# tlroy/thermalporous

Hardware: AMD Instinct MI355X
Metric: Newton steps/s, SPE10 60x220x85 two-phase (FGMRES its/s in config) (higher is better)
Workload: dtype f64; 1 GPU; BASELINE config 4: two-phase 3D SPE10-like 60x220x85, wells+heaters, pc_cptr, maxdt 0.1 day; grid 60x220x85 (synthetic default_rng(10) field); FGMRES rtol 1e-08; timed at dt = maxdt after an untimed spin-up along the reference's dt ramp; newton_its=84, fgmres_its=2689, failed_solves=0, slabs=none

## Files before the change

include/thermalporous_hip.h:

```cpp
#ifndef THERMALPOROUS_HIP_H
#define THERMALPOROUS_HIP_H

#include <stdint.h>

#ifdef __cplusplus
extern "C" {
#endif

typedef struct tp_ctx tp_ctx;

typedef struct tp_grid {
    int32_t n0, n1, n2;
    int32_t gn2, off2;
    double  h[3];
    int32_t gaxis;
    int32_t nphase;
    int32_t rank, nranks;
} tp_grid;

typedef struct tp_params {
    double ko, kw, kr, c_v_w, c_v_o, c_r, rho_r, p_inj, p_prod, T_inj, T_prod, API, p_ref, g,
           S_o, U, rate;
} tp_params;

// ... 54 lines not shown
int tp_set_field(tp_ctx *ctx, const char *name, const double *host, int64_t n);
int tp_finalize_fields(tp_ctx *ctx);
int tp_set_sources(tp_ctx *ctx, int32_t n, const tp_source *entries);

int tp_set_state(tp_ctx *ctx, const double *u_host);
int tp_get_state(tp_ctx *ctx, double *u_host);
int tp_set_old_state(tp_ctx *ctx, const double *u_host);
int tp_set_dt(tp_ctx *ctx, double dt);
int tp_get_old_state(tp_ctx *ctx, double *u_host);
int tp_restore_state(tp_ctx *ctx);
int tp_saturation_range(tp_ctx *ctx, double *smin, double *smax);
int tp_clamp_saturation(tp_ctx *ctx);

int tp_residual(tp_ctx *ctx, double *norm2);
int tp_jacobian(tp_ctx *ctx);
int tp_get_residual(tp_ctx *ctx, double *host);
int tp_export_jacobian(tp_ctx *ctx, double *host);
int tp_export_schur(tp_ctx *ctx, double *host);
int tp_well_rates(tp_ctx *ctx, double *rate, double *water_rate, double *oil_rate);

int tp_vec_create(tp_ctx *ctx, int32_t *id);
int tp_vec_set(tp_ctx *ctx, int32_t id, const double *host);
int tp_vec_get(tp_ctx *ctx, int32_t id, double *host);
int tp_vec_copy_residual(tp_ctx *ctx, int32_t id);

typedef void (*tp_ksp_monitor_fn)(int32_t its, double rnorm, const double *field_norms, int32_t nfields, void *user);
int tp_set_ksp_monitor(tp_ctx *ctx, tp_ksp_monitor_fn cb, void *user);

int tp_vec_create_batch(tp_ctx *ctx, int32_t n, int32_t *first_id);
int tp_vec_dot_batch(tp_ctx *ctx, int32_t first, int32_t n, int32_t w, double *out);
int tp_vec_axpy_batch(tp_ctx *ctx, int32_t first, int32_t n, const double *coef, int32_t w);
int tp_vec_norm2(tp_ctx *ctx, int32_t x, double *out);
int tp_spmv(tp_ctx *ctx, int32_t x, int32_t y);
int tp_pc_setup(tp_ctx *ctx);
int tp_pc_apply(tp_ctx *ctx, int32_t x, int32_t y);
int tp_stage1_update(tp_ctx *ctx);
int tp_stage1_apply(tp_ctx *ctx, int32_t x, int32_t y);
int tp_ilu0_factor(tp_ctx *ctx);
int tp_ilu0_solve(tp_ctx *ctx, int32_t x, int32_t y);
int tp_ilu_layout(tp_ctx *ctx, int32_t out[8]);
int tp_amg_setup(tp_ctx *ctx, int32_t which);
int tp_amg_vcycle(tp_ctx *ctx, int32_t which, int32_t field_b, int32_t b, int32_t field_x, int32_t x);
int tp_schur_apply(tp_ctx *ctx, int32_t x, int32_t y);

int tp_inner_stats(tp_ctx *ctx, int64_t *applies, int64_t *its, int64_t *unconverged);

int tp_fgmres(tp_ctx *ctx, int32_t b, int32_t x, int32_t *its, int32_t *reason, double *rnorm);
int tp_newton_solve(tp_ctx *ctx, tp_solve_info *info);

int tp_time_kernel(tp_ctx *ctx, int32_t which, int32_t reps, double *ms_avg);
int tp_amg_info(tp_ctx *ctx, int32_t which, int32_t *nlevels, double *op_complexity);
int tp_amg_trunc(tp_ctx *ctx, int32_t which, int32_t *level, double *ratio0);
int tp_amg_layout(tp_ctx *ctx, int32_t which, int32_t *dist_levels, int32_t *axes, int32_t cap, int32_t *naxes);

#ifdef __cplusplus
}
#endif
#endif
```

thermalporous_amd/csrc/tp_amg.hip:

```cpp
#include "tp_common.hpp"
#include <algorithm>
#include <cstdlib>

namespace tp {

template <class R>
struct StencilT {
    R *base;
    long slot_stride;
    __host__ __device__ const R *slot(int s) const { return base + (long)s * slot_stride; }
};

__device__ __forceinline__ void cell_ijk(const GridDev &g, long tid, int &i0, int &i1, int &i2) {
    const unsigned t = (unsigned)tid, np = (unsigned)g.np, n0 = (unsigned)g.n0;
    const unsigned q2 = t / np, rem = t - q2 * np, q1 = rem / n0;
    i2 = (int)q2;
    i1 = (int)q1;
    i0 = (int)(rem - q1 * n0);
}

template <class R>
__global__ void k_amg_weights(GridDev g, StencilT<R> A, int axis, double omega, R *wm, R *wp, R *invd,
                              unsigned long long *ratio_slots) {
    const long tid = (long)blockIdx.x * blockDim.x + threadIdx.x;
// ... 469 lines not shown
    if (tid >= Lf.g.nown) return;
    out[Lf.g.np + tid] = prolong_jacobi_cell(Lf, gc, b, x, ec, tid);
}

template <class R>
__global__ __launch_bounds__(256) void k_amg_restrict2(LevelDevT<R> L0, LevelDevT<R> L1, GridDev g2, const double *r,
                                                       double *rc) {
    const long tid = xcd_tid();
    if (tid >= g2.nown) return;
    rc[g2.np + tid] = restrict2_cell(L0, L1, g2, r, tid);
}
template <class R>
__global__ __launch_bounds__(256) void k_amg_prolong2_jacobi(LevelDevT<R> L0, LevelDevT<R> L1, GridDev g2, const double *b,
                                                             const double *e2, double *out) {
    const long tid = xcd_tid();
    if (tid >= L0.g.nown) return;
    out[L0.g.np + tid] = prolong2_jacobi_cell(L0, L1, g2, b, e2, tid);
}

template <class R>
__global__ __launch_bounds__(256) void k_amg_resid(LevelDevT<R> L, const double *__restrict__ b,
                                                   const double *__restrict__ x, double *__restrict__ r) {
    const long tid = xcd_tid();
    if (tid >= L.g.nown) return;
    r[L.g.np + tid] = resid_at(L, b, x, L.g.np + tid);
}
template <class R>
__global__ __launch_bounds__(256) void k_amg_restrict(LevelDevT<R> Lf, GridDev gc, const double *__restrict__ r,
                                                      double *__restrict__ rc) {
    const long tid = xcd_tid();
    if (tid >= gc.nown) return;
    rc[gc.np + tid] = restrict_cell(Lf, gc, r, tid);
}
template <class R>
__global__ __launch_bounds__(256) void k_amg_prolong_set(LevelDevT<R> Lf, GridDev gc, const double *__restrict__ ec,
                                                         double *__restrict__ out) {
    const long tid = xcd_tid();
    if (tid >= Lf.g.nown) return;
    int i0, i1, i2;
    cell_ijk(Lf.g, tid, i0, i1, i2);
    out[Lf.g.np + tid] = prolong_val<R, false>(Lf, gc, ec, i0, i1, i2);
}
template <class R>
__global__ __launch_bounds__(256) void k_amg_prolong_add(LevelDevT<R> Lf, GridDev gc, const double *__restrict__ ec,
                                                         double *x) {
    const long tid = xcd_tid();
    if (tid >= Lf.g.nown) return;
    int i0, i1, i2;
    cell_ijk(Lf.g, tid, i0, i1, i2);
    x[Lf.g.np + tid] += prolong_val<R, false>(Lf, gc, ec, i0, i1, i2);
}

template <class R>
__global__ __launch_bounds__(1024) void k_amg_tail(const LevelDevT<R> *lv, int l0, int nlev_all, int trunc, int ncoarse,
                                                   const double *Minv, const double *b_top, double *e_top,
                                                   int lds_doubles) {
    const int nlev = trunc >= 0 ? trunc + 1 : nlev_all;
    extern __shared__ double dyn[];
    constexpr int T = 1024;
    const int t = threadIdx.x;
    static_assert(sizeof(LevelDevT<R>) % sizeof(long) == 0, "LevelDev must be a whole number of words");
    __shared__ long slv_raw[40 * sizeof(LevelDevT<R>) / sizeof(long)];
    {
        const int wpl = (int)(sizeof(LevelDevT<R>) / sizeof(long));
        const long *src = reinterpret_cast<const long *>(lv);
        for (int i = l0 * wpl + t; i < nlev * wpl; i += T) slv_raw[i] = src[i];
        if (lds_doubles > 0)
            for (int i = t; i < 4 * lds_doubles; i += T) dyn[i] = 0.0;
        __syncthreads();
    }
    if (lds_doubles > 0) {
        if (t == 0) {
            LevelDevT<R> *w = reinterpret_cast<LevelDevT<R> *>(slv_raw);
            long off = 0;
            for (int l = l0; l < nlev; ++l) {
                w[l].b = dyn + off;
                w[l].e = dyn + lds_doubles + off;
                w[l].x = dyn + 2 * lds_doubles + off;
                w[l].x2 = dyn + 3 * lds_doubles + off;
                off += w[l].g.ntot;
            }
        }
        __syncthreads();
    }
    lv = reinterpret_cast<const LevelDevT<R> *>(slv_raw);
    {
        double sink = 0.0;
        for (int l = l0; l < nlev; ++l) {
            const LevelDevT<R> &L = lv[l];
            for (long i = L.g.np + t; i < L.g.np + L.g.nown; i += T) {
#pragma unroll
                for (int k = 0; k < 7; ++k) sink += (double)L.op.slot(k)[i];
                sink += (double)L.invd[i];
                if (L.axis >= 0) sink += (double)L.wm[i] + (double)L.wp[i];
            }
        }
        if (trunc < 0)
            for (int i = t; i < ncoarse * ncoarse; i += T) sink += Minv[i];
        if (sink == 1.2345678e-300) e_top[0] = sink;
    }
    for (int l = l0; l < nlev - 1; ++l) {
        const LevelDevT<R> L = lv[l];
        const GridDev gc = lv[l + 1].g;
        const double *b = (l == l0) ? b_top : L.b;
        double *rc = lv[l + 1].b;
        if (L.pre == 0) {
            for (long i = t; i < gc.nown; i += T) rc[gc.np + i] = restrict_cell(L, gc, b, i);
            __syncthreads();
            continue;
        }
        double *cur = L.x, *oth = L.x2;
        for (long i = t; i < L.g.nown; i += T)
            cur[L.g.np + i] = L.pre >= 2 ? pre2_cell(L, b, i) : L.invd[L.g.np + i] * b[L.g.np + i];
        __syncthreads();
        for (int k = 2; k < L.pre; ++k) {
            for (long i = t; i < L.g.nown; i += T) oth[L.g.np + i] = jacobi_cell(L, b, cur, i);
            __syncthreads();
            double *tmp = cur; cur = oth; oth = tmp;
        }
        for (long i = t; i < gc.nown; i += T) rc[gc.np + i] = resid_restrict_cell(L, gc, b, cur, i);
        __syncthreads();
    }
    {
        const LevelDevT<R> Lc = lv[nlev - 1];
        const double *b = (nlev - 1 == l0) ? b_top : Lc.b;
        double *e = (nlev - 1 == l0) ? e_top : Lc.e;
        if (trunc >= 0) {
            for (long i = t; i < Lc.g.nown; i += T) e[Lc.g.np + i] = pre2_cell(Lc, b, i);
            __syncthreads();
        } else {
        const int grp = t >> 4, gl = t & 15;
        for (int r = grp; r < ncoarse; r += T >> 4) {
            double s = 0.0;
            for (int q = gl; q < ncoarse; q += 16) s += Minv[(long)r * ncoarse + q] * b[Lc.g.np + q];
            s += __shfl_xor(s, 8, 64);
            s += __shfl_xor(s, 4, 64);
            s += __shfl_xor(s, 2, 64);
            s += __shfl_xor(s, 1, 64);
            if (gl == 0) e[Lc.g.np + r] = s;
        }
        __syncthreads();
        }
    }
    for (int l = nlev - 2; l >= l0; --l) {
        const LevelDevT<R> L = lv[l];
        const GridDev gc = lv[l + 1].g;
        const double *b = (l == l0) ? b_top : L.b;
        double *out = (l == l0) ? e_top : L.e;
        const double *ec = lv[l + 1].e;
        const int extra = L.pre >= 2 ? L.pre - 2 : 0;
        const double *src = L.pre == 0 ? nullptr : ((extra % 2 == 0) ? L.x : L.x2);
        if (L.post == 0) {
            for (long i = t; i < L.g.nown; i += T) {
                int i0, i1, i2;
                cell_ijk(L.g, i, i0, i1, i2);
                out[L.g.np + i] = prolong_val(L, gc, ec, i0, i1, i2);
            }
            __syncthreads();
            continue;
        }
        double *dst = (L.post == 1) ? out : (src == L.x ? L.x2 : L.x);
        for (long i = t; i < L.g.nown; i += T) dst[L.g.np + i] = prolong_jacobi_cell(L, gc, b, src, ec, i);
        __syncthreads();
        for (int k = 1; k < L.post; ++k) {
            src = dst;
            dst = (k == L.post - 1) ? out : (src == L.x ? L.x2 : L.x);
            for (long i = t; i < L.g.nown; i += T) dst[L.g.np + i] = jacobi_cell(L, b, src, i);
            __syncthreads();
        }
    }
}

std::vector<std::pair<int, int>> rank_slabs(const tp_ctx *c) {
    std::vector<std::pair<int, int>> slabs(c->dist ? c->grid.nranks : 0);
    for (size_t r = 0; r < slabs.size(); ++r) slab_of(c, (int)r, slabs[r].first, slabs[r].second);
    return slabs;
}

AmgPlan amg_plan(const GridDev &g0, const double strength[3], const tp_options &o, int me,
                 const std::vector<std::pair<int, int>> &slabs, long gather_cells, long tail_cells) {
    AmgPlan P;
    int m[3] = {g0.n0, g0.n1, g0.n2};
    {
        int n[3] = {m[0], m[1], m[2]};
        double s[3];
        for (int a = 0; a < 3; ++a) s[a] = n[a] > 1 ? strength[a] : -1.0;
        while ((long)n[0] * n[1] * n[2] > std::max(1, o.amg_min_cells) && P.sched.size() < 40) {
            int best = -1;
            for (int a = 0; a < 3; ++a)
                if (n[a] > 1 && (best < 0 || s[a] > s[best])) best = a;
            if (best < 0) break;
            P.sched.push_back(best);
            n[best] = (n[best] + 1) / 2;
            for (int q = 0; q < 3; ++q) s[q] = (q == best) ? s[q] * 0.5 : s[q] * 2.0;
        }
    }
    std::vector<std::pair<int, int>> cur = slabs;
    if (cur.empty()) cur = {{0, m[2]}};
    bool still = !slabs.empty() && gather_cells >= 0;
    const int nu = std::max(1, o.amg_nu);
    for (size_t l = 0; l <= P.sched.size(); ++l) {
        AmgPlan::Level L;
        if (still) {
            int minp = 1 << 30;
            for (auto &q : cur) minp = std::min(minp, q.second - q.first);
            still = (long)m[0] * m[1] * m[2] > gather_cells && minp >= 2 && l < P.sched.size();
            if (still) P.dist_levels = (int)l + 1;
        }
        P.ranges.push_back(cur);
        L.g = still ? make_grid(m[0], m[1], cur[me].second - cur[me].first, m[2], cur[me].first)
                    : make_grid(m[0], m[1], m[2], m[2], 0);
        const bool full = (int)l < o.amg_full_levels;
        const bool small = L.g.np * (long)L.g.gn2 <= 1024;
        L.pre = full ? nu : std::max(0, o.amg_coarse_pre);
        L.post = full ? nu : std::max(1, small ? o.amg_tail_post : o.amg_coarse_post);
        if (o.amg_mid_skip && !full && !small && (((int)l - o.amg_full_levels) & 1)) { L.pre = 0; L.post = 0; }
        if (l < P.sched.size()) {
            L.axis = P.sched[l];
            m[L.axis] = (m[L.axis] + 1) / 2;
            if (L.axis == 2)
                for (auto &q : cur) q = {(q.first + 1) / 2, (q.second + 1) / 2};
        }
        P.lv.push_back(L);
    }
    P.tail_level = (int)P.lv.size() - 1;
// ... 19 lines not shown
}

void amg_build(tp_ctx *c, Amg *&amg, const GridDev &g0, const double strength[3], long gather_cells) {
    delete amg;
    amg = new Amg();
    c->graph_epoch++;
    amg->single = c->opt.amg_single != 0;
    const long tail_cells = getenv("TP_AMG_TAIL_CELLS") ? atol(getenv("TP_AMG_TAIL_CELLS")) : 1024;
    amg->plan = amg_plan(g0, strength, c->opt, c->dist ? c->grid.rank : 0, rank_slabs(c), gather_cells, tail_cells);
    for (const AmgPlan::Level &P : amg->plan.lv) {
        AmgLevel *L = new AmgLevel();
        L->g = P.g;
        L->axis = P.axis;
        amg->lv.push_back(L);
    }
    {
        auto pad = [](size_t v) { return (v + 31) & ~(size_t)31; };
        size_t total = 0;
        for (size_t l = 0; l < amg->lv.size(); ++l) {
            const size_t nt = pad((size_t)amg->lv[l]->g.ntot);
            total += ((l > 0 || amg->single) ? 7 : 0) * nt + 5 * nt + (amg->lv[l]->axis >= 0 ? 2 * nt : 0);
        }
        amg->arena.alloc(total);
        double *q = amg->arena.p;
        auto take = [&](DBuf<double> &d, size_t nd, size_t step) { d.view(q, nd); q += step; };
        for (size_t l = 0; l < amg->lv.size(); ++l) {
            AmgLevel *L = amg->lv[l];
            const size_t nt = (size_t)L->g.ntot, ntp = pad(nt);
            if (l > 0 || amg->single) {
                take(L->A, 7 * nt, 7 * ntp);
                L->op.base = L->A.p;
                L->op.slot_stride = (long)nt;
            }
            take(L->invd, nt, ntp);
            take(L->b, nt, ntp); take(L->x, nt, ntp); take(L->x2, nt, ntp); take(L->e, nt, ntp);
            if (L->axis >= 0) { take(L->wm, nt, ntp); take(L->wp, nt, ntp); }
        }
    }
    amg->ncoarse = (int)amg->lv.back()->g.nown;
    TP_REQUIRE(amg->ncoarse <= 1024, "coarsest AMG grid too large for the dense solve");
    amg->ratio_dev.alloc(64 * 8);
    TP_HIP(hipHostMalloc((void **)&amg->ratio_host, 64 * 8 * sizeof(double)));
    TP_HIP(hipEventCreateWithFlags(&amg->ev_ratio, hipEventDisableTiming));
    amg->coarse_inv.alloc((size_t)2 * amg->ncoarse * amg->ncoarse);
    amg->fuse_below = getenv("TP_AMG_FUSE_BELOW") ? atol(getenv("TP_AMG_FUSE_BELOW")) : 200000;
    amg->lvdev.alloc(amg->lv.size() * sizeof(LevelDevT<double>));
    long tot = 0;
    for (size_t l = (size_t)amg->plan.tail_level; l < amg->lv.size(); ++l) tot += amg->lv[l]->g.ntot;
    const bool lds_on = !(getenv("TP_AMG_TAIL_LDS") && atoi(getenv("TP_AMG_TAIL_LDS")) == 0);
    amg->tail_lds = (lds_on && 4 * tot * (long)sizeof(double) <= 120 * 1024) ? (int)tot : 0;
    if (getenv("TP_DEBUG")) fprintf(stderr, "[tp] amg tail: level %d of %zu, %ld doubles per vector set, lds %d\n", amg->plan.tail_level, amg->lv.size(), tot, amg->tail_lds);
    if (amg->tail_lds > 0) {
        const int bytes = 120 * 1024;
        TP_HIP(hipFuncSetAttribute(reinterpret_cast<const void *>(&k_amg_tail<double>),
                                   hipFuncAttributeMaxDynamicSharedMemorySize, bytes));
        TP_HIP(hipFuncSetAttribute(reinterpret_cast<const void *>(&k_amg_tail<float>),
                                   hipFuncAttributeMaxDynamicSharedMemorySize, bytes));
    }
}

template <class R>
__global__ void k_amg_import(GridDev g, Stencil A0, R *out) {
    const long tid = (long)blockIdx.x * blockDim.x + threadIdx.x;
    if (tid >= g.nown) return;
    const long c = g.np + tid;
#pragma unroll
    for (int s = 0; s < 7; ++s) out[(long)s * g.ntot + c] = (R)A0.slot(s)[c];
}

template <class R>
static void setup_impl(tp_ctx *c, Amg *amg, const Stencil &A0) {
    AmgLevel *L0 = amg->lv[0];
    const int lg = amg->plan.dist_levels;
    if (sizeof(R) == sizeof(double)) {
        L0->op = A0;
    } else {
        hipLaunchKernelGGL(k_amg_import<R>, grid_for(L0->g.nown), dim3(256), 0, c->stream, L0->g, A0, (R *)L0->A.p);
        L0->op.base = L0->A.p;
        L0->op.slot_stride = L0->g.ntot;
    }
    const int nratio = c->opt.amg_dom_tau > 0.0 ? std::min({c->opt.amg_full_levels, (int)amg->lv.size() - 1, 8}) : 0;
    if (nratio > 0) TP_HIP(hipMemsetAsync(amg->ratio_dev.p, 0, sizeof(double) * 64 * nratio, c->stream));
    for (size_t l = 0; l < amg->lv.size(); ++l) {
        AmgLevel *L = amg->lv[l];
        const StencilT<R> op{(R *)L->op.base, L->op.slot_stride};
        const bool want_ratio = (int)l < nratio;
        hipLaunchKernelGGL(k_amg_weights<R>, grid_for(L->g.nown, want_ratio ? 1024 : 256), dim3(want_ratio ? 1024 : 256), 0, c->stream, L->g, op, L->axis,
                           c->opt.amg_omega, (R *)L->wm.p, (R *)L->wp.p, (R *)L->invd.p,
                           (int)l < nratio ? (unsigned long long *)amg->ratio_dev.p + 64 * l : (unsigned long long *)nullptr);
        if ((int)l < lg) {
            halo_exchange_raw(c, L->g, L->invd.p, 1, 0, sizeof(R));
            halo_exchange_raw(c, L->g, L->wm.p, 1, 0, sizeof(R));
            halo_exchange_raw(c, L->g, L->wp.p, 1, 0, sizeof(R));
            if (L->axis == 2) halo_exchange_raw(c, L->g, L->op.base, 7, (size_t)L->op.slot_stride * sizeof(R), sizeof(R));
        }
        if (L->axis >= 0) {
            AmgLevel *Lc = amg->lv[l + 1];
            const AmgPlan::View cv = amg->plan.coarse_view((int)l, c->grid.rank);
            hipLaunchKernelGGL(k_amg_coarsen<R>, grid_for(cv.g.nown), dim3(256), 0, c->stream, L->g, cv.g, op, L->axis,
                               (const R *)L->wm.p, (const R *)L->wp.p, (R *)Lc->A.p + cv.off, Lc->g.ntot);
            if ((int)l + 1 == lg)
                gather_ranges(c, Lc->A.p, Lc->g.np, amg->plan.ranges[lg], 7, (size_t)Lc->g.ntot * sizeof(R), sizeof(R));
        }
    }
    AmgLevel *Lc = amg->lv.back();
    const int n = amg->ncoarse;
    const StencilT<R> opc{(R *)Lc->op.base, Lc->op.slot_stride};
    static const bool skip_dense = getenv("TP_EXP_SKIP_DENSE") && atoi(getenv("TP_EXP_SKIP_DENSE")) == 1;
    if (skip_dense && amg->dense_done) {
    } else if (n <= 64) {
        const bool mfma = !(getenv("TP_AMG_DENSE_MFMA") && atoi(getenv("TP_AMG_DENSE_MFMA")) == 0);
        if (mfma) {
            const int bytes = (64 * 128 + 4 * 128 + 64 * 4 + 16) * (int)sizeof(double);
            TP_HIP(hipFuncSetAttribute(reinterpret_cast<const void *>(&k_amg_dense_inverse_mfma<R>),
                                       hipFuncAttributeMaxDynamicSharedMemorySize, bytes));
            hipLaunchKernelGGL(k_amg_dense_inverse_mfma<R>, dim3(1), dim3(1024), bytes, c->stream, Lc->g, opc, n,
                               amg->coarse_inv.p + (size_t)n * n);
        } else {
            hipLaunchKernelGGL(k_amg_dense_inverse_lds<R>, dim3(1), dim3(1024), 0, c->stream, Lc->g, opc, n,
                               amg->coarse_inv.p + (size_t)n * n);
        }
    }
    else
        hipLaunchKernelGGL(k_amg_dense_inverse<R>, dim3(1), dim3(256), 0, c->stream, Lc->g, opc, n, amg->coarse_inv.p,
                           amg->coarse_inv.p + (size_t)n * n);
    amg->dense_done = true;
    std::vector<LevelDevT<R>> h;
    for (size_t l = 0; l < amg->lv.size(); ++l) h.push_back(dev_of<R>(amg, (int)l));
    amg->lvhost.assign((const char *)h.data(), (const char *)h.data() + h.size() * sizeof(LevelDevT<R>));
    TP_HIP(hipMemcpyAsync(amg->lvdev.p, amg->lvhost.data(), amg->lvhost.size(), hipMemcpyHostToDevice, c->stream));
    if (nratio > 0) {
        if (lg > 0) allreduce_max(c, amg->ratio_dev.p, 64 * nratio);
        TP_HIP(hipMemcpyAsync(amg->ratio_host, amg->ratio_dev.p, sizeof(double) * 64 * nratio, hipMemcpyDeviceToHost, c->stream));
        TP_HIP(hipEventRecord(amg->ev_ratio, c->stream));
        amg->ratio_pending = true;
    } else if (amg->trunc != -1) {
        amg->trunc = -1;
        c->graph_epoch++;
    }
    TP_HIP(hipGetLastError());
}

bool amg_resolve_trunc(tp_ctx *c, Amg *amg) {
    if (!amg || !amg->ratio_pending) return false;
    TP_HIP(hipEventSynchronize(amg->ev_ratio));
    amg->ratio_pending = false;
    const int nratio = std::min({c->opt.amg_full_levels, (int)amg->lv.size() - 1, 8});
    int t = -1;
    for (int l = 0; l < nratio; ++l) {
        double r = 0.0;
        for (int q = 0; q < 64; ++q) r = std::max(r, amg->ratio_host[64 * l + q]);
        if (l == 0) amg->ratio0 = r;
        if (r <= c->opt.amg_dom_tau) { t = l; break; }
    }
    const bool changed = t != amg->trunc;
    amg->trunc = t;
    return changed;
}

void amg_setup(tp_ctx *c, Amg *amg, const Stencil &A0) {
    static_assert(sizeof(LevelDevT<float>) == sizeof(LevelDevT<double>), "descriptor size");
    if (amg->single) setup_impl<float>(c, amg, A0);
    else setup_impl<double>(c, amg, A0);
}

template <class R>
static void vcycle_impl(tp_ctx *c, Amg *amg, const double *b, double *x) {
    const int nlev = (int)amg->lv.size(), lt = amg->plan.tail_level, lg = amg->plan.dist_levels;
    const int trunc = amg->trunc;
    const int ltop = (trunc >= 0 && trunc < lt) ? trunc : lt;
    const dim3 bl(256);
    std::vector<double *> xs(nlev, nullptr);
    static const bool pair_on = !(getenv("TP_AMG_PAIR") && atoi(getenv("TP_AMG_PAIR")) == 0);
    auto paired = [&](int l) {
        if (!pair_on || l < lg || l + 2 > lt || amg->lv[l]->g.nown >= amg->fuse_below) return false;
        if (trunc >= 0 && l + 2 > trunc) return false;
        const AmgPlan::Level &A = amg->plan.lv[l], &B = amg->plan.lv[l + 1];
        return A.pre == 0 && A.post >= 1 && B.pre == 0 && B.post == 0;
    };
    auto hx = [&](int l, const double *v) {
        if (l < lg) halo_exchange(c, amg->lv[l]->g, const_cast<double *>(v), 1, 0);
    };
    for (int l = 0; l < ltop; ++l) {
        AmgLevel *L = amg->lv[l];
        AmgLevel *Lc = amg->lv[l + 1];
        const LevelDevT<R> Ld = dev_of<R>(amg, l);
        const AmgPlan::View cv = amg->plan.coarse_view(l, c->grid.rank);
        const double *bl_ = (l == 0) ? b : L->b.p;
        double *bc = Lc->b.p + cv.off;
        const dim3 gr = xcd_grid(L->g.nown);
        const bool slab_axis = l < lg && L->axis == 2;
        if (paired(l)) {
            AmgLevel *L2 = amg->lv[l + 2];
            hipLaunchKernelGGL(k_amg_restrict2<R>, xcd_grid(L2->g.nown), bl, 0, c->stream, Ld,
                               dev_of<R>(amg, l + 1), L2->g, bl_, L2->b.p);
            ++l;
            continue;
        }
        if (Ld.pre == 0) {
            if (slab_axis) hx(l, bl_);
            hipLaunchKernelGGL(k_amg_restrict<R>, xcd_grid(cv.g.nown), bl, 0, c->stream, Ld, cv.g, bl_, bc);
        } else {
            double *cur = L->x.p, *oth = L->x2.p;
            if (Ld.pre >= 2) hx(l, bl_);
            hipLaunchKernelGGL(k_amg_pre<R>, gr, bl, 0, c->stream, Ld, bl_, Ld.pre >= 2 ? 1 : 0, cur);
            for (int k = 2; k < Ld.pre; ++k) {
                hx(l, cur);
                hipLaunchKernelGGL(k_amg_jacobi<R>, gr, bl, 0, c->stream, Ld, bl_, (const double *)cur, oth);
                std::swap(cur, oth);
            }
            xs[l] = cur;
            hx(l, cur);
            if (slab_axis || L->g.nown >= amg->fuse_below) {
                hipLaunchKernelGGL(k_amg_resid<R>, gr, bl, 0, c->stream, Ld, bl_, (const double *)cur, oth);
                if (slab_axis) hx(l, oth);
                hipLaunchKernelGGL(k_amg_restrict<R>, xcd_grid(cv.g.nown), bl, 0, c->stream, Ld, cv.g, (const double *)oth, bc);
            } else {
                hipLaunchKernelGGL(k_amg_resid_restrict<R>, xcd_grid(cv.g.nown), bl, 0, c->stream, Ld, cv.g, bl_,
                                   (const double *)cur, bc);
            }
        }
        if (l + 1 == lg)
            gather_ranges(c, Lc->b.p, Lc->g.np, amg->plan.ranges[lg], 1, 0, sizeof(double));
    }
    if (trunc >= 0 && trunc < lt) {
        AmgLevel *L = amg->lv[trunc];
        const double *bt = (trunc == 0) ? b : L->b.p;
        double *et = (trunc == 0) ? x : L->e.p;
        hx(trunc, bt);
        hipLaunchKernelGGL(k_amg_pre<R>, xcd_grid(L->g.nown), bl, 0, c->stream, dev_of<R>(amg, trunc), bt, 1, et);
    } else {
        AmgLevel *Lt = amg->lv[lt];
        const double *bt = (lt == 0) ? b : Lt->b.p;
        double *et = (lt == 0) ? x : Lt->e.p;
        const int n = amg->ncoarse;
        hipLaunchKernelGGL(k_amg_tail<R>, dim3(1), dim3(1024), (size_t)4 * amg->tail_lds * sizeof(double), c->stream,
                           (const LevelDevT<R> *)amg->lvdev.p, lt, nlev, trunc, n,
                           (const double *)(amg->coarse_inv.p + (size_t)n * n), bt, et, amg->tail_lds);
    }
    for (int l = ltop - 1; l >= 0; --l) {
        AmgLevel *L = amg->lv[l];
        AmgLevel *Lc = amg->lv[l + 1];
        const LevelDevT<R> Ld = dev_of<R>(amg, l);
        const AmgPlan::View cv = amg->plan.coarse_view(l, c->grid.rank);
        const double *bl_ = (l == 0) ? b : L->b.p;
        double *out = (l == 0) ? x : L->e.p;
        const double *ec = Lc->e.p + cv.off;
        const dim3 gr = xcd_grid(L->g.nown);
        double *src = xs[l];
        double *dst = (Ld.post == 1) ? out : (src == L->x.p ? L->x2.p : L->x.p);
        if (l >= 1 && paired(l - 1)) continue;
        if (paired(l)) {
            AmgLevel *L2 = amg->lv[l + 2];
            hipLaunchKernelGGL(k_amg_prolong2_jacobi<R>, gr, bl, 0, c->stream, Ld, dev_of<R>(amg, l + 1), L2->g, bl_,
                               (const double *)L2->e.p, dst);
            for (int k = 1; k < Ld.post; ++k) {
                src = dst;
                dst = (k == Ld.post - 1) ? out : (src == L->x.p ? L->x2.p : L->x.p);
                hipLaunchKernelGGL(k_amg_jacobi<R>, gr, bl, 0, c->stream, Ld, bl_, (const double *)src, dst);
            }
            continue;
        }
        hx(l + 1, Lc->e.p);
        if (Ld.post == 0) {
            hipLaunchKernelGGL(k_amg_prolong_set<R>, gr, bl, 0, c->stream, Ld, cv.g, ec, out);
            continue;
        }
        if (src && L->g.nown >= amg->fuse_below) {
            hipLaunchKernelGGL(k_amg_prolong_add<R>, gr, bl, 0, c->stream, Ld, cv.g, ec, src);
            hx(l, src);
            hipLaunchKernelGGL(k_amg_jacobi<R>, gr, bl, 0, c->stream, Ld, bl_, (const double *)src, dst);
        } else {
            hipLaunchKernelGGL(k_amg_prolong_jacobi<R>, gr, bl, 0, c->stream, Ld, cv.g, bl_, (const double *)src, ec, dst);
        }
        for (int k = 1; k < Ld.post; ++k) {
            src = dst;
            dst = (k == Ld.post - 1) ? out : (src == L->x.p ? L->x2.p : L->x.p);
            hx(l, src);
            hipLaunchKernelGGL(k_amg_jacobi<R>, gr, bl, 0, c->stream, Ld, bl_, (const double *)src, dst);
        }
    }
    TP_HIP(hipGetLastError());
}

void amg_vcycle(tp_ctx *c, Amg *amg, const double *b, double *x) {
    TP_REQUIRE(amg && !amg->lv.empty(), "AMG not set up");
    TP_REQUIRE(!amg->ratio_pending, "amg_resolve_trunc must run after a set-up and before the first cycle");
    TP_REQUIRE(x != amg->lv[0]->x.p && x != amg->lv[0]->x2.p && b != x, "aliasing in amg_vcycle");
    if (amg->single) vcycle_impl<float>(c, amg, b, x);
    else vcycle_impl<double>(c, amg, b, x);
}
// ... 3 lines not shown
```

thermalporous_amd/csrc/tp_api.hip:

```cpp
#include "tp_common.hpp"
#include <rccl/rccl.h>
#include <cmath>
#include <algorithm>
#include <map>
#include <utility>
#include <mutex>
#include <condition_variable>

namespace tp {

static thread_local std::string g_err;
void set_error(const std::string &msg) { g_err = msg; }

#define TP_NCCL(call)                                                                          \
    do {                                                                                       \
        ncclResult_t r_ = (call);                                                              \
        if (r_ != ncclSuccess)                                                                 \
            throw tp::Error(std::string(#call) + " failed: " + ncclGetErrorString(r_));        \
    } while (0)

struct LocalGroup {
    int n = 0;
    std::mutex mu;
    std::condition_variable cv;
// ... 808 lines not shown
    for (int i = 0; i < reps; ++i) run();
    TP_HIP(hipEventRecord(c->ev1, c->stream));
    TP_HIP(hipEventSynchronize(c->ev1));
    float ms = 0.f;
    TP_HIP(hipEventElapsedTime(&ms, c->ev0, c->ev1));
    *ms_avg = (double)ms / reps;
    TP_API_END
}

static const AmgPlan &plan_of(tp_ctx *c, int which) {
    if (which == 2) {
        TP_REQUIRE(c->bamg, "system AMG hierarchy not built");
        return c->bamg->plan;
    }
    Amg *amg = which == 0 ? c->amg_p : c->amg_T;
    TP_REQUIRE(amg, "AMG hierarchy not built");
    return amg->plan;
}

int tp_amg_info(tp_ctx *c, int32_t which, int32_t *nlevels, double *op_complexity) {
    TP_API_BEGIN
    const AmgPlan &P = plan_of(c, which);
    if (nlevels) *nlevels = (int)P.lv.size();
    double s = 0.0, s0 = 0.0;
    for (size_t l = 0; l < P.lv.size(); ++l) {
        const GridDev &g = P.lv[l].g;
        const double cells = (double)g.np * g.gn2;
        s += cells;
        if (l == 0) s0 = cells;
    }
    if (op_complexity) *op_complexity = which == 2 ? 0.0 : s / s0;
    TP_API_END
}

int tp_amg_trunc(tp_ctx *c, int32_t which, int32_t *level, double *ratio0) {
    TP_API_BEGIN
    Amg *amg = which == 0 ? c->amg_p : c->amg_T;
    TP_REQUIRE(amg, "AMG hierarchy not built");
    resolve_cycle_shapes(c);
    if (level) *level = amg->trunc;
    if (ratio0) *ratio0 = amg->ratio0;
    TP_API_END
}

int tp_amg_layout(tp_ctx *c, int32_t which, int32_t *dist_levels, int32_t *axes, int32_t cap, int32_t *naxes) {
    TP_API_BEGIN
    const AmgPlan &P = plan_of(c, which);
    if (dist_levels) *dist_levels = P.dist_levels;
    if (naxes) *naxes = (int)P.sched.size();
    for (int i = 0; axes && i < cap && i < (int)P.sched.size(); ++i) axes[i] = P.sched[i];
    TP_API_END
}

int tp_ilu_layout(tp_ctx *c, int32_t out[8]) {
    TP_API_BEGIN
    TP_REQUIRE(c && out, "null argument");
    ilu_layout(c, out);
    TP_API_END
}

}
```

thermalporous_amd/csrc/tp_common.hpp:

```cpp
#pragma once
#include <hip/hip_runtime.h>
#include <cstdint>
#include <cstdio>
#include <cstring>
#include <string>
#include <vector>
#include <stdexcept>
#include <functional>
#include "../../include/thermalporous_hip.h"

struct ncclComm;

namespace tp {
struct LocalGroup;

void set_error(const std::string &msg);

struct Error : std::runtime_error {
    using std::runtime_error::runtime_error;
};

#define TP_HIP(call)                                                                             \
    do {                                                                                         \
        hipError_t e_ = (call);                                                                  \
// ... 92 lines not shown
    ~DBuf() { free(); }
    DBuf() = default;
    DBuf(const DBuf &) = delete;
    DBuf &operator=(const DBuf &) = delete;
};

struct AmgPlan {
    struct Level {
        GridDev g;
        int axis = -1;
        int pre = 0, post = 0;
    };
    std::vector<int> sched;
    std::vector<Level> lv;
    int dist_levels = 0;
    int tail_level = 0;
    std::vector<std::vector<std::pair<int, int>>> ranges;
    struct View {
        GridDev g;
        long off;
    };
    View coarse_view(int l, int rank) const {
        const GridDev &gc = lv[l + 1].g;
        if (l + 1 < dist_levels || l >= dist_levels) return {gc, 0};
        const auto &q = ranges[l + 1][rank];
        return {make_grid(gc.n0, gc.n1, q.second - q.first, gc.n2, q.first), gc.np * q.first};
    }
};

struct AmgLevel {
    GridDev g;
    DBuf<double> A;
    Stencil op;
    DBuf<double> invd;
    DBuf<double> wm, wp;
    DBuf<double> b, x, x2, r, e;
    int axis = -1;
};

struct Amg {
    AmgPlan plan;
    DBuf<double> arena;
    std::vector<AmgLevel *> lv;
    DBuf<double> coarse_inv;
    int ncoarse = 0;
    bool single = false;
    int tail_lds = 0;
    long fuse_below = 200000;
    DBuf<double> ratio_dev;
    double *ratio_host = nullptr;
    hipEvent_t ev_ratio = nullptr;
    bool ratio_pending = false;
    int trunc = -1;
    bool dense_done = false;
    double ratio0 = 0.0;
    DBuf<char> lvdev;
    std::vector<char> lvhost;
    ~Amg() {
        for (auto *l : lv) delete l;
        if (ratio_host) (void)hipHostFree(ratio_host);
        if (ev_ratio) (void)hipEventDestroy(ev_ratio);
    }
};

struct BAmgLevel {
    GridDev g;
    DBuf<double> A;
    BStencil op;
    DBuf<double> invD;
    DBuf<double> wm, wp;
    DBuf<double> b, x, x2, r, e;
    int axis = -1;
    int pre = 0, post = 0;
};

struct BAmg {
    AmgPlan plan;
    int nb = 2;
    std::vector<BAmgLevel *> lv;
    DBuf<double> dense;
    int ncoarse = 0;
    long fuse_below = 0;
    DBuf<char> lvdev;
    std::vector<char> lvhost;
    ~BAmg() { for (auto *l : lv) delete l; }
};

struct InnerOp {
    GridDev g;
    Stencil A[2][2];
};
struct InnerWork {
    DBuf<double> V, Z;
    DBuf<double> partial;
    DBuf<double> state;
    DBuf<long long> stats;
};

struct IluData {
    int t0 = 0, t1 = 8, t2 = 8, nt0 = 0, nt1 = 0, nt2 = 0, ntiles = 0, nsteps = 0;
    DBuf<double> fwd, bwd, ytmp;
    DBuf<double> jt;
    long slots = 0;
    bool mw = false;
    int levels = 0;
    DBuf<double> fwdp, bwdp;
    DBuf<int> pref;
    int ptot = 0;
// ... 143 lines not shown
```

thermalporous_amd/engine.py:

```python
import ctypes as C
import os

import numpy as np

_LIB = None
_LIBPATH = os.path.join(os.path.dirname(os.path.abspath(__file__)), "libthermalporous_hip.so")


class EngineError(RuntimeError):
    pass


class tp_grid(C.Structure):
    _fields_ = [("n0", C.c_int32), ("n1", C.c_int32), ("n2", C.c_int32), ("gn2", C.c_int32), ("off2", C.c_int32),
                ("h", C.c_double*3), ("gaxis", C.c_int32), ("nphase", C.c_int32), ("rank", C.c_int32),
                ("nranks", C.c_int32)]


class tp_params(C.Structure):
    _names = ("ko", "kw", "kr", "c_v_w", "c_v_o", "c_r", "rho_r", "p_inj", "p_prod", "T_inj", "T_prod", "API",
              "p_ref", "g", "S_o", "U", "rate")
    _fields_ = [(k, C.c_double) for k in _names]


class tp_source(C.Structure):
    _fields_ = [("cell", C.c_int64), ("kind", C.c_int32), ("constant_rate", C.c_int32), ("wt", C.c_double),
                ("bhp", C.c_double), ("max_rate", C.c_double), ("WI", C.c_double)]


class tp_options(C.Structure):
    _fields_ = [("pc_kind", C.c_int32), ("decoup", C.c_int32), ("ksp_rtol", C.c_double), ("ksp_atol", C.c_double),
                ("ksp_max_it", C.c_int32), ("ksp_restart", C.c_int32), ("snes_rtol", C.c_double),
                ("snes_atol", C.c_double), ("snes_stol", C.c_double), ("snes_max_it", C.c_int32),
                ("amg_omega", C.c_double), ("amg_nu", C.c_int32), ("amg_min_cells", C.c_int32),
                ("ilu_t1", C.c_int32), ("ilu_t2", C.c_int32), ("ilu_t0", C.c_int32),
                ("amg_full_levels", C.c_int32), ("amg_coarse_pre", C.c_int32), ("amg_coarse_post", C.c_int32),
                ("amg_mid_skip", C.c_int32), ("amg_tail_post", C.c_int32), ("amg_single", C.c_int32), ("schur_a11", C.c_int32), ("amg_gather_cells", C.c_int32), ("amg_dom_tau", C.c_double),
                ("ilu_levels", C.c_int32), ("fs_additive", C.c_int32), ("ilu_whole", C.c_int32),
                ("ilu_block", C.c_int32*3),
                ("s1_ksp", C.c_int32), ("s1_max_it", C.c_int32), ("s1_rtol", C.c_double), ("s1_atol", C.c_double)]


class tp_solve_info(C.Structure):
    _fields_ = [("nits", C.c_int32), ("lits", C.c_int32), ("reason", C.c_int32), ("last_ksp_reason", C.c_int32),
                ("fnorm0", C.c_double), ("fnorm", C.c_double), ("vcycles", C.c_int32)]


API_SYMBOLS = (
    "tp_last_error", "tp_version", "tp_create", "tp_destroy", "tp_set_options", "tp_comm_unique_id", "tp_comm_init",
    "tp_local_group_create", "tp_local_group_destroy", "tp_comm_init_local",
    "tp_set_field", "tp_finalize_fields", "tp_set_sources", "tp_set_state", "tp_get_state", "tp_set_old_state",
    "tp_set_dt", "tp_get_old_state", "tp_restore_state", "tp_saturation_range", "tp_clamp_saturation",
    "tp_residual", "tp_jacobian", "tp_get_residual", "tp_export_jacobian", "tp_export_schur",
    "tp_well_rates", "tp_vec_create", "tp_vec_create_batch", "tp_vec_dot_batch", "tp_vec_axpy_batch", "tp_vec_norm2", "tp_set_ksp_monitor", "tp_vec_set", "tp_vec_get", "tp_vec_copy_residual", "tp_spmv", "tp_pc_setup",
    "tp_pc_apply", "tp_stage1_update", "tp_stage1_apply", "tp_ilu0_factor", "tp_ilu0_solve", "tp_ilu_layout", "tp_amg_setup",
    "tp_amg_vcycle", "tp_schur_apply", "tp_fgmres", "tp_newton_solve", "tp_time_kernel", "tp_amg_info", "tp_amg_layout", "tp_amg_trunc",
    "tp_inner_stats",
)

DEFAULT_OPTS = dict(
    pc="cpr", decoup="No",
    ksp_rtol=1e-7, ksp_atol=1e-50, ksp_max_it=200, ksp_restart=200,
    snes_rtol=1e-8, snes_atol=1e-50, snes_stol=1e-8, snes_max_it=15,
    amg_omega=0.9,
    amg_min_cells=64, amg_nu=2, amg_full_levels=3, amg_coarse_pre=0, amg_coarse_post=1, amg_mid_skip=True, amg_tail_post=2, amg_single=False,
    amg_dom_tau=0.25,
    amg_gather_cells=600000,
    schur_a11=False,
    fs_additive=False,
    schur_selfp=False,
    ilu_tile=None,
    ilu_levels=0,
    bjacobi_blocks=None,
    ilu_block=None,
    ilu_whole=False,
    s1_ksp="preonly",
    s1_max_it=1,
    s1_rtol=0.0, s1_atol=0.0,
)

def default_ilu_tile(n, nslabs=1, ncu=256):
    n0, n1, n2 = (int(v) for v in n)
    if n2 == 1:
        return (-(-n0//max(1, -(-n0//24))), 32, 1)
    n2l = -(-n2//max(1, int(nslabs)))
    best = None
    for t1 in range(min(4, n1), min(16, n1) + 1):
        for t2 in range(min(4, n2l), min(16, n2l) + 1):
            lanes = t1*t2
            if lanes > 64 or (lanes < 32 and (t1 < min(16, n1) or t2 < min(16, n2l))):
                continue
            tiles = -(-n1//t1)*-(-n2l//t2)
            cost = -(-tiles//ncu)*(n0 + t1 + t2 - 2)*lanes*(1.0 + 0.01*abs(t1 - t2))
            key = (cost, -lanes, abs(t1 - t2))
            if best is None or key < best[0]:
                best = (key, (1 << 30, t1, t2))
    if best is None:
        return (1 << 30, min(n1, 8), min(n2l, 8))
    return best[1]


def whole_ilu_tile(n, nslabs=1):
    n0, n1, n2 = (int(v) for v in n)
    t = default_ilu_tile(n, nslabs=nslabs)
    if n2 == 1:
        return t
    return (-(-n0//max(1, -(-n0//16))), t[1], t[2])


def block_ilu_tile(block):
# ... 327 lines not shown

    def spmv(self, x, y):
        self._ck(self.lib.tp_spmv(self.ctx, self.vec(x), self.vec(y)))

    def pc_setup(self):
        self._ck(self.lib.tp_pc_setup(self.ctx))

    def pc_apply(self, x, y):
        self._ck(self.lib.tp_pc_apply(self.ctx, self.vec(x), self.vec(y)))

    def stage1_apply(self, x, y):
        self._ck(self.lib.tp_stage1_apply(self.ctx, self.vec(x), self.vec(y)))

    def ilu_solve(self, x, y):
        self._ck(self.lib.tp_ilu0_solve(self.ctx, self.vec(x), self.vec(y)))

    def schur_apply(self, x, y):
        self._ck(self.lib.tp_schur_apply(self.ctx, self.vec(x), self.vec(y)))

    def vec_axpby(self, out, a, x, b, y):
        self.vec_set(out, a*self._full(self.vec_get(x)) + b*self._full(self.vec_get(y)))

    def _full(self, owned):
        if self.nranks != 1:
            raise EngineError("host-side vector algebra is only available on single-slab engines")
        return owned

    def amg_vcycle(self, which, b, fb, x, fx):
        self._ck(self.lib.tp_amg_vcycle(self.ctx, which, fb, self.vec(b), fx, self.vec(x)))

    def fgmres(self, b, x):
        its, reason, rn = C.c_int32(), C.c_int32(), C.c_double()
        self._ck(self.lib.tp_fgmres(self.ctx, self.vec(b), self.vec(x), C.byref(its), C.byref(reason), C.byref(rn)))
        return its.value, reason.value, rn.value

    def copy_residual_to(self, name):
        self._ck(self.lib.tp_vec_copy_residual(self.ctx, self.vec(name)))

    def time_kernel(self, which, reps):
        ms = C.c_double()
        self._ck(self.lib.tp_time_kernel(self.ctx, which, reps, C.byref(ms)))
        return ms.value

    def amg_info(self, which=0):
        nl, oc = C.c_int32(), C.c_double()
        self._ck(self.lib.tp_amg_info(self.ctx, which, C.byref(nl), C.byref(oc)))
        return nl.value, oc.value

    def amg_trunc(self, which=0):
        lv, r0 = C.c_int32(), C.c_double()
        self._ck(self.lib.tp_amg_trunc(self.ctx, which, C.byref(lv), C.byref(r0)))
        return lv.value, r0.value

    def amg_layout(self, which=0):
        nd, na = C.c_int32(), C.c_int32()
        axes = (C.c_int32*64)()
        self._ck(self.lib.tp_amg_layout(self.ctx, which, C.byref(nd), axes, 64, C.byref(na)))
        return nd.value, [axes[i] for i in range(min(na.value, 64))]

    def ilu_layout(self):
        out = (C.c_int32*8)()
        self._ck(self.lib.tp_ilu_layout(self.ctx, out))
        return dict(block=(out[0], out[1], out[2]), nblocks=out[3], ntiles=out[4], ndiag=out[5], max_tiles_per_launch=out[6],
                    launches=out[7])

    def inner_stats(self):
        a, i, u = C.c_int64(), C.c_int64(), C.c_int64()
        self._ck(self.lib.tp_inner_stats(self.ctx, C.byref(a), C.byref(i), C.byref(u)))
        return a.value, i.value, u.value

    def newton_solve(self):
        info = tp_solve_info()
        self._ck(self.lib.tp_newton_solve(self.ctx, C.byref(info)))
        self.last = dict(nits=info.nits, lits=info.lits, reason=info.reason, fnorm=info.fnorm, fnorm0=info.fnorm0,
                         ksp_reason=info.last_ksp_reason, vcycles=info.vcycles)
        return self.last

    def close(self):
        if self.ctx:
            self.lib.tp_destroy(self.ctx)
            self.ctx = C.c_void_p()

    def __del__(self):
        try:
            self.close()
        except Exception:
            pass
```

Baseline: 27.97 Newton steps/s.

## Replace single-block AMG tail sweeps with a precomputed dense tail operator

At each AMG set-up, the linear map from tail-level RHS to tail correction is formed explicitly by running the tail sweeps on each unit vector in a multi-block build kernel. Each V-cycle then applies this dense matrix with a wave-per-row matvec instead of the serial single-workgroup tail kernel. This removes the latency-bound one-block tail from every preconditioner apply, at the cost of n tail solves per set-up and n^2 storage. It only applies when the tail level has at most 1024 cells and no truncation is active, and it also drops the old debug skip-dense path.

```diff
diff --git a/include/thermalporous_hip.h b/include/thermalporous_hip.h
--- a/include/thermalporous_hip.h
+++ b/include/thermalporous_hip.h
@@ -130,6 +130,7 @@
 int tp_amg_info(tp_ctx *ctx, int32_t which, int32_t *nlevels, double *op_complexity);
 int tp_amg_trunc(tp_ctx *ctx, int32_t which, int32_t *level, double *ratio0);
 int tp_amg_layout(tp_ctx *ctx, int32_t which, int32_t *dist_levels, int32_t *axes, int32_t cap, int32_t *naxes);
+int tp_amg_tail_info(tp_ctx *ctx, int32_t which, int64_t out[6]);
 
 #ifdef __cplusplus
 }
diff --git a/thermalporous_amd/csrc/tp_amg.hip b/thermalporous_amd/csrc/tp_amg.hip
--- a/thermalporous_amd/csrc/tp_amg.hip
+++ b/thermalporous_amd/csrc/tp_amg.hip
@@ -545,53 +545,10 @@
 }
 
 template <class R>
-__global__ __launch_bounds__(1024) void k_amg_tail(const LevelDevT<R> *lv, int l0, int nlev_all, int trunc, int ncoarse,
-                                                   const double *Minv, const double *b_top, double *e_top,
-                                                   int lds_doubles) {
-    const int nlev = trunc >= 0 ? trunc + 1 : nlev_all;
-    extern __shared__ double dyn[];
+__device__ __forceinline__ void tail_sweeps(const LevelDevT<R> *lv, int l0, int nlev, int trunc, int ncoarse,
+                                            const double *Minv, const double *b_top, double *e_top) {
     constexpr int T = 1024;
     const int t = threadIdx.x;
-    static_assert(sizeof(LevelDevT<R>) % sizeof(long) == 0, "LevelDev must be a whole number of words");
-    __shared__ long slv_raw[40 * sizeof(LevelDevT<R>) / sizeof(long)];
-    {
-        const int wpl = (int)(sizeof(LevelDevT<R>) / sizeof(long));
-        const long *src = reinterpret_cast<const long *>(lv);
-        for (int i = l0 * wpl + t; i < nlev * wpl; i += T) slv_raw[i] = src[i];
-        if (lds_doubles > 0)
-            for (int i = t; i < 4 * lds_doubles; i += T) dyn[i] = 0.0;
-        __syncthreads();
-    }
-    if (lds_doubles > 0) {
-        if (t == 0) {
-            LevelDevT<R> *w = reinterpret_cast<LevelDevT<R> *>(slv_raw);
-            long off = 0;
-            for (int l = l0; l < nlev; ++l) {
-                w[l].b = dyn + off;
-                w[l].e = dyn + lds_doubles + off;
-                w[l].x = dyn + 2 * lds_doubles + off;
-                w[l].x2 = dyn + 3 * lds_doubles + off;
-                off += w[l].g.ntot;
-            }
-        }
-        __syncthreads();
-    }
-    lv = reinterpret_cast<const LevelDevT<R> *>(slv_raw);
-    {
-        double sink = 0.0;
-        for (int l = l0; l < nlev; ++l) {
-            const LevelDevT<R> &L = lv[l];
-            for (long i = L.g.np + t; i < L.g.np + L.g.nown; i += T) {
-#pragma unroll
-                for (int k = 0; k < 7; ++k) sink += (double)L.op.slot(k)[i];
-                sink += (double)L.invd[i];
-                if (L.axis >= 0) sink += (double)L.wm[i] + (double)L.wp[i];
-            }
-        }
-        if (trunc < 0)
-            for (int i = t; i < ncoarse * ncoarse; i += T) sink += Minv[i];
-        if (sink == 1.2345678e-300) e_top[0] = sink;
-    }
     for (int l = l0; l < nlev - 1; ++l) {
         const LevelDevT<R> L = lv[l];
         const GridDev gc = lv[l + 1].g;
@@ -664,6 +621,99 @@
     }
 }
 
+struct TailBuild {
+    double *Tm = nullptr, *scratch = nullptr;
+    int vec_doubles = 0;
+};
+template <class R, bool BUILD>
+__global__ __launch_bounds__(1024) void k_amg_tail(const LevelDevT<R> *lv, int l0, int nlev_all, int trunc, int ncoarse,
+                                                   const double *Minv, const double *b_top, double *e_top,
+                                                   int lds_doubles, TailBuild tb) {
+    const int nlev = trunc >= 0 ? trunc + 1 : nlev_all;
+    extern __shared__ double dyn[];
+    constexpr int T = 1024;
+    const int t = threadIdx.x;
+    static_assert(sizeof(LevelDevT<R>) % sizeof(long) == 0, "LevelDev must be a whole number of words");
+    __shared__ long slv_raw[40 * sizeof(LevelDevT<R>) / sizeof(long)];
+    {
+        const int wpl = (int)(sizeof(LevelDevT<R>) / sizeof(long));
+        const long *src = reinterpret_cast<const long *>(lv);
+        for (int i = l0 * wpl + t; i < nlev * wpl; i += T) slv_raw[i] = src[i];
+        if (lds_doubles > 0)
+            for (int i = t; i < 4 * lds_doubles; i += T) dyn[i] = 0.0;
+        __syncthreads();
+    }
+    if (lds_doubles > 0 || BUILD) {
+        if (t == 0) {
+            LevelDevT<R> *w = reinterpret_cast<LevelDevT<R> *>(slv_raw);
+            double *base = dyn;
+            long vd = lds_doubles;
+            if (BUILD && lds_doubles == 0) { vd = tb.vec_doubles; base = tb.scratch + (long)blockIdx.x * 4 * vd; }
+            long off = 0;
+            for (int l = l0; l < nlev; ++l) {
+                w[l].b = base + off;
+                w[l].e = base + vd + off;
+                w[l].x = base + 2 * vd + off;
+                w[l].x2 = base + 3 * vd + off;
+                off += w[l].g.ntot;
+            }
+        }
+        __syncthreads();
+    }
+    lv = reinterpret_cast<const LevelDevT<R> *>(slv_raw);
+    {
+        double sink = 0.0;
+        for (int l = l0; l < nlev; ++l) {
+            const LevelDevT<R> &L = lv[l];
+            for (long i = L.g.np + t; i < L.g.np + L.g.nown; i += T) {
+#pragma unroll
+                for (int k = 0; k < 7; ++k) sink += (double)L.op.slot(k)[i];
+                sink += (double)L.invd[i];
+                if (L.axis >= 0) sink += (double)L.wm[i] + (double)L.wp[i];
+            }
+        }
+        if (trunc < 0)
+            for (int i = t; i < ncoarse * ncoarse; i += T) sink += Minv[i];
+        if (sink == 1.2345678e-300) (BUILD ? tb.Tm : e_top)[0] = sink;
+    }
+    if constexpr (!BUILD) {
+        tail_sweeps(lv, l0, nlev, trunc, ncoarse, Minv, b_top, e_top);
+    } else {
+        double *ub = lv[l0].b, *ue = lv[l0].e;
+        const long np = lv[l0].g.np;
+        const int n = (int)lv[l0].g.nown;
+        for (int j = blockIdx.x; j < n; j += gridDim.x) {
+            if (t == 0) ub[np + j] = 1.0;
+            __syncthreads();
+            tail_sweeps(lv, l0, nlev, trunc, ncoarse, Minv, ub, ue);
+            for (int i = t; i < n; i += T) tb.Tm[(long)i * n + j] = ue[np + i];
+            if (t == 0) ub[np + j] = 0.0;
+            __syncthreads();
+        }
+    }
+}
+
+template <int NK>
+__global__ __launch_bounds__(TP_BLOCK) void k_amg_tail_dense(const double *__restrict__ Tm, int n, long np,
+                                                             const double *__restrict__ b, double *__restrict__ e) {
+    const int row = (int)blockIdx.x * (TP_BLOCK / 64) + ((int)threadIdx.x >> 6), lane = threadIdx.x & 63;
+    if (row >= n) return;
+    const double *tr = Tm + (long)row * n;
+    double tv[NK], bv[NK];
+#pragma unroll
+    for (int k = 0; k < NK; ++k) {
+        const int q = lane + 64 * k, qc = q < n ? q : 0;
+        tv[k] = tr[qc];
+        bv[k] = b[np + qc];
+    }
+    double s = 0.0;
+#pragma unroll
+    for (int k = 0; k < NK; ++k) s += (lane + 64 * k < n) ? tv[k] * bv[k] : 0.0;
+#pragma unroll
+    for (int o = 32; o > 0; o >>= 1) s += __shfl_xor(s, o, 64);
+    if (lane == 0) e[np + row] = s;
+}
+
 std::vector<std::pair<int, int>> rank_slabs(const tp_ctx *c) {
     std::vector<std::pair<int, int>> slabs(c->dist ? c->grid.nranks : 0);
     for (size_t r = 0; r < slabs.size(); ++r) slab_of(c, (int)r, slabs[r].first, slabs[r].second);
@@ -789,10 +839,21 @@
     if (getenv("TP_DEBUG")) fprintf(stderr, "[tp] amg tail: level %d of %zu, %ld doubles per vector set, lds %d\n", amg->plan.tail_level, amg->lv.size(), tot, amg->tail_lds);
     if (amg->tail_lds > 0) {
         const int bytes = 120 * 1024;
-        TP_HIP(hipFuncSetAttribute(reinterpret_cast<const void *>(&k_amg_tail<double>),
-                                   hipFuncAttributeMaxDynamicSharedMemorySize, bytes));
-        TP_HIP(hipFuncSetAttribute(reinterpret_cast<const void *>(&k_amg_tail<float>),
-                                   hipFuncAttributeMaxDynamicSharedMemorySize, bytes));
+        const void *fns[4] = {reinterpret_cast<const void *>(&k_amg_tail<double, false>),
+                              reinterpret_cast<const void *>(&k_amg_tail<float, false>),
+                              reinterpret_cast<const void *>(&k_amg_tail<double, true>),
+                              reinterpret_cast<const void *>(&k_amg_tail<float, true>)};
+        for (const void *f : fns) TP_HIP(hipFuncSetAttribute(f, hipFuncAttributeMaxDynamicSharedMemorySize, bytes));
+    }
+    const long ntop = amg->lv[amg->plan.tail_level]->g.nown;
+    amg->tail_vec = tot;
+    amg->tdense_eligible = (int)amg->lv.size() - amg->plan.tail_level >= 2 && ntop <= 1024;
+    if (amg->tdense_eligible) {
+        amg->tdense.alloc((size_t)ntop * ntop);
+        amg->tdense_groups = (int)ntop;
+        if (amg->tail_lds == 0) {
+            amg->tdense_groups = (int)std::max(1L, std::min(ntop, (32L << 20) / (4 * tot * (long)sizeof(double))));
+        }
     }
 }
 
@@ -803,6 +864,33 @@
     const long c = g.np + tid;
 #pragma unroll
     for (int s = 0; s < 7; ++s) out[(long)s * g.ntot + c] = (R)A0.slot(s)[c];
+}
+
+static bool tail_dense_needed(const Amg *amg, bool shape_resolved) {
+    return amg->tdense_on && shape_resolved && amg->trunc < 0 && amg->tdense_stamp != amg->setup_id;
+}
+
+static void tail_dense_build(tp_ctx *c, Amg *amg) {
+    if (amg->tail_lds == 0 && !amg->tdense_scratch.p)
+        amg->tdense_scratch.alloc((size_t)amg->tdense_groups * 4 * amg->tail_vec);
+    const int lt = amg->plan.tail_level, nlev = (int)amg->lv.size(), n = amg->ncoarse;
+    TailBuild tb;
+    tb.Tm = amg->tdense.p;
+    tb.scratch = amg->tdense_scratch.p;
+    tb.vec_doubles = (int)amg->tail_vec;
+    const size_t lds = (size_t)4 * amg->tail_lds * sizeof(double);
+    const double *Minv = amg->coarse_inv.p + (size_t)n * n;
+    if (amg->single)
+        hipLaunchKernelGGL((k_amg_tail<float, true>), dim3(amg->tdense_groups), dim3(1024), lds, c->stream,
+                           (const LevelDevT<float> *)amg->lvdev.p, lt, nlev, -1, n, Minv, (const double *)nullptr,
+                           (double *)nullptr, amg->tail_lds, tb);
+    else
+        hipLaunchKernelGGL((k_amg_tail<double, true>), dim3(amg->tdense_groups), dim3(1024), lds, c->stream,
+                           (const LevelDevT<double> *)amg->lvdev.p, lt, nlev, -1, n, Minv, (const double *)nullptr,
+                           (double *)nullptr, amg->tail_lds, tb);
+    TP_HIP(hipGetLastError());
+    amg->tdense_stamp = amg->setup_id;
+    amg->tdense_builds++;
 }
 
 template <class R>
@@ -843,9 +931,7 @@
     AmgLevel *Lc = amg->lv.back();
     const int n = amg->ncoarse;
     const StencilT<R> opc{(R *)Lc->op.base, Lc->op.slot_stride};
-    static const bool skip_dense = getenv("TP_EXP_SKIP_DENSE") && atoi(getenv("TP_EXP_SKIP_DENSE")) == 1;
-    if (skip_dense && amg->dense_done) {
-    } else if (n <= 64) {
+    if (n <= 64) {
         const bool mfma = !(getenv("TP_AMG_DENSE_MFMA") && atoi(getenv("TP_AMG_DENSE_MFMA")) == 0);
         if (mfma) {
             const int bytes = (64 * 128 + 4 * 128 + 64 * 4 + 16) * (int)sizeof(double);
@@ -861,7 +947,6 @@
     else
         hipLaunchKernelGGL(k_amg_dense_inverse<R>, dim3(1), dim3(256), 0, c->stream, Lc->g, opc, n, amg->coarse_inv.p,
                            amg->coarse_inv.p + (size_t)n * n);
-    amg->dense_done = true;
     std::vector<LevelDevT<R>> h;
     for (size_t l = 0; l < amg->lv.size(); ++l) h.push_back(dev_of<R>(amg, (int)l));
     amg->lvhost.assign((const char *)h.data(), (const char *)h.data() + h.size() * sizeof(LevelDevT<R>));
@@ -875,6 +960,14 @@
         amg->trunc = -1;
         c->graph_epoch++;
     }
+    amg->setup_id++;
+    const bool dense_env = !(getenv("TP_AMG_TAIL_DENSE") && atoi(getenv("TP_AMG_TAIL_DENSE")) == 0);
+    const bool dense = dense_env && amg->tdense_eligible && amg->plan.tail_level >= nratio;
+    if (dense != amg->tdense_on) {
+        amg->tdense_on = dense;
+        c->graph_epoch++;
+    }
+    if (tail_dense_needed(amg, nratio == 0 || amg->setup_id > 1)) tail_dense_build(c, amg);
     TP_HIP(hipGetLastError());
 }
 
@@ -892,6 +985,7 @@
     }
     const bool changed = t != amg->trunc;
     amg->trunc = t;
+    if (tail_dense_needed(amg, true)) tail_dense_build(c, amg);
     return changed;
 }
 
@@ -971,9 +1065,22 @@
         const double *bt = (lt == 0) ? b : Lt->b.p;
         double *et = (lt == 0) ? x : Lt->e.p;
         const int n = amg->ncoarse;
-        hipLaunchKernelGGL(k_amg_tail<R>, dim3(1), dim3(1024), (size_t)4 * amg->tail_lds * sizeof(double), c->stream,
-                           (const LevelDevT<R> *)amg->lvdev.p, lt, nlev, trunc, n,
-                           (const double *)(amg->coarse_inv.p + (size_t)n * n), bt, et, amg->tail_lds);
+        if (amg->tdense_on) {
+            TP_REQUIRE(trunc < 0 && amg->tdense_stamp == amg->setup_id, "the dense AMG tail was not formed for the last set-up");
+            const int nt = (int)Lt->g.nown;
+            const dim3 gd((unsigned)((nt + TP_BLOCK / 64 - 1) / (TP_BLOCK / 64))), bd(TP_BLOCK);
+            const double *Tm = amg->tdense.p;
+            if (nt <= 256) hipLaunchKernelGGL(k_amg_tail_dense<4>, gd, bd, 0, c->stream, Tm, nt, Lt->g.np, bt, et);
+            else if (nt <= 512) hipLaunchKernelGGL(k_amg_tail_dense<8>, gd, bd, 0, c->stream, Tm, nt, Lt->g.np, bt, et);
+            else if (nt <= 768) hipLaunchKernelGGL(k_amg_tail_dense<12>, gd, bd, 0, c->stream, Tm, nt, Lt->g.np, bt, et);
+            else hipLaunchKernelGGL(k_amg_tail_dense<16>, gd, bd, 0, c->stream, Tm, nt, Lt->g.np, bt, et);
+            amg->tdense_applies++;
+        } else {
+            hipLaunchKernelGGL((k_amg_tail<R, false>), dim3(1), dim3(1024), (size_t)4 * amg->tail_lds * sizeof(double), c->stream,
+                               (const LevelDevT<R> *)amg->lvdev.p, lt, nlev, trunc, n,
+                               (const double *)(amg->coarse_inv.p + (size_t)n * n), bt, et, amg->tail_lds, TailBuild());
+            amg->tail_launches++;
+        }
     }
     for (int l = ltop - 1; l >= 0; --l) {
         AmgLevel *L = amg->lv[l];
diff --git a/thermalporous_amd/csrc/tp_api.hip b/thermalporous_amd/csrc/tp_api.hip
--- a/thermalporous_amd/csrc/tp_api.hip
+++ b/thermalporous_amd/csrc/tp_api.hip
@@ -884,6 +884,20 @@
     TP_API_END
 }
 
+int tp_amg_tail_info(tp_ctx *c, int32_t which, int64_t out[6]) {
+    TP_API_BEGIN
+    Amg *amg = which == 0 ? c->amg_p : c->amg_T;
+    TP_REQUIRE(amg && out, "AMG hierarchy not built");
+    resolve_cycle_shapes(c);
+    out[0] = amg->tdense_on ? 1 : 0;
+    out[1] = amg->plan.tail_level;
+    out[2] = amg->lv[amg->plan.tail_level]->g.nown;
+    out[3] = amg->tdense_builds;
+    out[4] = amg->tdense_applies;
+    out[5] = amg->tail_launches;
+    TP_API_END
+}
+
 int tp_ilu_layout(tp_ctx *c, int32_t out[8]) {
     TP_API_BEGIN
     TP_REQUIRE(c && out, "null argument");
diff --git a/thermalporous_amd/csrc/tp_common.hpp b/thermalporous_amd/csrc/tp_common.hpp
--- a/thermalporous_amd/csrc/tp_common.hpp
+++ b/thermalporous_amd/csrc/tp_common.hpp
@@ -168,8 +168,16 @@
     hipEvent_t ev_ratio = nullptr;
     bool ratio_pending = false;
     int trunc = -1;
-    bool dense_done = false;
     double ratio0 = 0.0;
+    DBuf<double> tdense;
+    DBuf<double> tdense_scratch;
+    long tail_vec = 0;
+    int tdense_groups = 0;
+    bool tdense_eligible = false;
+    bool tdense_on = false;
+    uint64_t setup_id = 0;
+    uint64_t tdense_stamp = ~(uint64_t)0;
+    long tdense_builds = 0, tdense_applies = 0, tail_launches = 0;
     DBuf<char> lvdev;
     std::vector<char> lvhost;
     ~Amg() {
diff --git a/thermalporous_amd/engine.py b/thermalporous_amd/engine.py
--- a/thermalporous_amd/engine.py
+++ b/thermalporous_amd/engine.py
@@ -55,7 +55,7 @@
     "tp_well_rates", "tp_vec_create", "tp_vec_create_batch", "tp_vec_dot_batch", "tp_vec_axpy_batch", "tp_vec_norm2", "tp_set_ksp_monitor", "tp_vec_set", "tp_vec_get", "tp_vec_copy_residual", "tp_spmv", "tp_pc_setup",
     "tp_pc_apply", "tp_stage1_update", "tp_stage1_apply", "tp_ilu0_factor", "tp_ilu0_solve", "tp_ilu_layout", "tp_amg_setup",
     "tp_amg_vcycle", "tp_schur_apply", "tp_fgmres", "tp_newton_solve", "tp_time_kernel", "tp_amg_info", "tp_amg_layout", "tp_amg_trunc",
-    "tp_inner_stats",
+    "tp_inner_stats", "tp_amg_tail_info",
 )
 
 DEFAULT_OPTS = dict(
@@ -489,6 +489,11 @@
         self._ck(self.lib.tp_amg_trunc(self.ctx, which, C.byref(lv), C.byref(r0)))
         return lv.value, r0.value
 
+    def amg_tail_info(self, which=0):
+        out = (C.c_int64*6)()
+        self._ck(self.lib.tp_amg_tail_info(self.ctx, which, out))
+        return dict(dense=bool(out[0]), tail_level=out[1], n=out[2], builds=out[3], dense_applies=out[4], tail_launches=out[5])
+
     def amg_layout(self, which=0):
         nd, na = C.c_int32(), C.c_int32()
         axes = (C.c_int32*64)()
```

Result: faster. 29.18 Newton steps/s (median of 6 runs) (+4.3%).
